# arturxe2/T-DEED

Hardware: AMD Instinct MI355X
Metric: clips/sec (L=100, 224^2, bf16) forward, per-frame logits (higher is better)
Workload: dtype bf16; 1 GPU; rny002_b8: rny002_gsf + ed_sgp_mixer n_layers=2 ks=7, L=100, 224x224, batch 8/GPU, inference forward, random-init weights; clips_per_gpu=8, parallelism=dp1 (clip-sharded, no collective), hip_graph=True, batches_in_flight=3, sub_batches_per_batch=1, dist_backend=none, dist_ranks=1, self_launched=False

## Files before the change

include/tdeed_hip.h:

```cpp
#ifndef TDEED_HIP_H
#define TDEED_HIP_H
#include <stdint.h>
#ifdef __cplusplus
extern "C" {
#endif

enum { TDEED_F32 = 0, TDEED_BF16 = 1 };
enum { TDEED_ACT_NONE = 0, TDEED_ACT_RELU = 1, TDEED_ACT_GELU = 2 };
enum { TDEED_OK = 0, TDEED_ERR_ARG = -1, TDEED_ERR_LAUNCH = -2, TDEED_ERR_RUNTIME = -3 };

const char* tdeed_last_error(void);
int tdeed_abi_version(void);
int tdeed_device_info(int dev, char* name64, int* n_cu, int* is_gfx950);

int tdeed_stem_fwd(const void* frames , int frames_f32,
                   int N, int H, int W, int crop_top, int crop_left,
                   int crop_h, int crop_w, int flip ,
                   const unsigned char* flip_mask ,
                   const float* w ,
                   const float* scale , const float* shift , void* out,
                   int relu , int dtype, void* stream);

int tdeed_stem_mfma_parts(int crop_h, int crop_w);
int tdeed_stem_mfma_fwd(const void* frames, int frames_f32, int N, int H, int W, int crop_top, int crop_left, int crop_h,
// ... 22 lines not shown
                      int gather_ho, int gather_wo, void* C2, long ldc2, int n2, int dtype, void* stream);

int tdeed_gemm_ws_sc_fits(int K, int Ks, int N, int dtype);
int tdeed_gemm_ws_sc_fwd(const void* A, long lda, const void* A0, long lda0, int k0, const float* a_scale,
                         int a_scale_rows, int M, int K, int N, const void* Wfrag, const float* scale,
                         const float* shift, const void* As, long ldas, int Ks, const void* Wsfrag,
                         const float* sscale, const float* sshift, int act, void* C, long ldc, int gather_stride,
                         int gather_hi, int gather_wi, int gather_ho, int gather_wo, void* C2, long ldc2, int n2,
                         int dtype, void* stream);

int tdeed_gconv3x3_parts(int Hi, int Wi, int C, int stride, int dtype);
int tdeed_gconv3x3_mfma_fits(int Hi, int Wi, int C, int stride);
int tdeed_gconv3x3_fwd(const void* x, int N, int Hi, int Wi, int C, int gw, int stride,
                       const float* w, const void* wfrag, const float* scale, const float* shift,
                       void* y, float* pooled, float* pooled_sq, const float* in_a, const float* in_b,
                       int relu , int dtype,
                       void* stream);

int tdeed_gemm_splitk_splits(int K);
int tdeed_gemm_splitk_partials(const void* A, long lda, int M, int K, int N, const void* W, long ldw, float* workspace,
                               void* stream);
int tdeed_gemm_splitk_fwd(const void* A, long lda, int M, int K, int N, const void* W, long ldw, const float* scale,
                          const float* shift, const void* R, long ldr, int act, void* C, long ldc,
                          float* workspace, void* stream);

int tdeed_se_gate_mfma_fits(int C, int R);
int tdeed_se_gate_mfma_fwd(const float* pooled, int n_parts, float inv_cnt, int N, int C, int R, const void* w1f,
                           const float* b1, const void* w2f, const float* b2, float* gate, void* stream);

int tdeed_gemm_rs_fits(int M, int K, int N);
int tdeed_gemm_rs_fwd(const void* A, long lda, const void* A0, long lda0, int k0, const float* a_scale, int a_scale_rows,
                      int M, int K, int N, const void* Wfrag, const float* scale, const float* shift, const void* R, long ldr,
                      int act, void* C, long ldc, void* C2, long ldc2, int n2, void* stream);

int tdeed_gemm_rs_grid(int M);
int tdeed_gemm_rs_stats_fwd(const void* A, long lda, const void* A0, long lda0, int k0, int M, int K, int N, const void* Wfrag,
                            void* C, long ldc, float* colpart, void* stream);

int tdeed_c1_gconv_set_debug(void* buf);
int tdeed_c1_gconv_fits(int Hi, int Wi, int Cin, int C, int stride);
int tdeed_c1_gconv_slab_tiles(int Hi, int Wi, int C, int stride);
int tdeed_c1_gconv_fwd(const void* x, const void* G, int Fp, int N, int Hi, int Wi, int Cin, int C, int gw, int stride,
                       const void* w1f, const float* s1, const float* h1, const void* wfrag, const float* scale,
                       const float* shift, void* y, float* pooled, void* stream);
int tdeed_c1_gconv_set_form(int form);
int tdeed_c1_gconv_slab_loop_fits(int Hi, int Wi, int Cin, int C, int stride);
int tdeed_c1_gconv_workgroups(int N, int Hi, int Wi, int Cin, int C, int stride);

int tdeed_c1_gconv_c3in_fits(int Hi, int Wi, int Cp, int C);
int tdeed_c1_gconv_c3in_fwd(const void* y2p, const void* scp, const float* gate, const void* w3f, const float* s3,
                            const float* h3, void* xs2, int N, int Hi, int Wi, int Cp, int C, int gw, const void* w1f,
                            const float* s1, const float* h1, const void* wfrag, const float* scale, const float* shift,
                            void* y, float* pooled, void* stream);

int tdeed_bneck_fits(int h, int w, int C, int R);
int tdeed_bneck_set_debug(void* buf);
int tdeed_bneck_fwd(const void* x, const void* G, int Fp, int N, int h, int w, int C, const void* w1f, const float* s1,
                    const float* h1, const void* w2f, const float* s2, const float* h2, const void* se_w1f,
                    const float* se_b1, const void* se_w2f, const float* se_b2, int R, const void* w3f, const float* s3,
                    const float* h3, void* out, void* out2, int n2,
                    int w2_tap_major ,
                    void* stream);
int tdeed_bneck_qtail_fits(int h, int w, int C, int F);
int tdeed_bneck_gs_fwd(const void* x, const void* gx, int ldx, const float* gate, const float* ysum, const float* xsum,
                       const float* cw1, const float* cb1, const float* cw2, const float* cb2, int T, int F, int Fp, int N,
                       int h, int w, int C, const void* w1f, const float* s1, const float* h1, const void* w2f,
                       const float* s2, const float* h2, const void* se_w1f, const float* se_b1, const void* se_w2f,
                       const float* se_b2, int R, const void* w3f, const float* s3, const float* h3, void* out, void* out2,
                       int n2, int w2_tap_major, const void* q_wqf, const float* q_bn, int q_F, float* Q, void* stream);


int tdeed_se_gate_fwd(const float* pooled, int n_parts, float inv_cnt, int N, int C, int R,
                      const float* w1t, const float* b1, const float* w2t, const float* b2,
                      float* gate, void* stream);

int tdeed_se_gate_bf16_fwd(const float* pooled, int n_parts, float inv_cnt, int N, int C, int R,
                           const void* w1p, const float* b1, const void* w2p, const float* b2,
                           float* gate, void* stream);

int tdeed_gsf_gate_fwd(const void* x, int B, int T, int h, int w, int C, int F,
                       const float* bn_scale, const float* bn_shift,
                       const float* wq ,
                       const void* wqf ,
                       const float* b3d ,
                       float* Q , float* gate, float* ysum, float* xsum,
                       int dtype, void* stream);
int tdeed_gsf_gate_sums_fwd(const void* x, int B, int T, int h, int w, int C, int F, const float* b3d, const float* Q,
                            float* gate, float* ysum, float* xsum, void* stream);
int tdeed_gsf_weight_fwd(const float* ysum, const float* xsum, int B, int T, int F, int hw,
                         const float* cw1 , const float* cb1, const float* cw2,
                         const float* cb2, float* fw , void* stream);
int tdeed_gsf_apply_fwd(const void* x, const float* gate, const float* fw , int B,
                        int T, int h, int w, int C, int F, int Fp, void* out, int dtype,
                        void* stream);

int tdeed_gsf_apply_fused_fwd(const void* x, const float* gate, const float* ysum, const float* xsum,
                              const float* cw1, const float* cb1, const float* cw2, const float* cb2, int B,
                              int T, int h, int w, int C, int F, int Fp, void* out, int dtype, void* stream);
int tdeed_gsf_blend_src_fwd(const void* x, const float* gate, const float* ysum, const float* xsum,
                            const float* cw1, const float* cb1, const float* cw2, const float* cb2, int B,
                            int T, int h, int w, int C, int F, int Fp, void* out, int dtype, void* stream);

int tdeed_avgpool_posenc_fwd(const void* x, int B, int T, int hw, int C, const float* temp_enc,
                             void* feat, float* rowstat, int dtype, int dtype_out , void* stream);

int tdeed_layernorm_fwd(const void* x, long ldx, int rows, int C, const float* w, const float* b,
// ... 248 lines not shown
```

t-deed_amd/_lib.py:

```python
import ctypes
import os
from ctypes import c_int, c_long, c_float, c_double, c_void_p, c_char_p, c_uint64, POINTER

import torch

CSRC = os.path.join(os.path.dirname(os.path.abspath(__file__)), "csrc")
LIB_PATH = os.path.join(CSRC, "libtdeed_hip.so")

F32, BF16 = 0, 1
ACT_NONE, ACT_RELU, ACT_GELU = 0, 1, 2


class HipLibraryMissing(RuntimeError):
    pass


class HipCallError(RuntimeError):
    pass


P = c_void_p
_SIGS = {
    "tdeed_abi_version": ([], c_int),
    "tdeed_device_info": ([c_int, c_char_p, POINTER(c_int), POINTER(c_int)], c_int),
    "tdeed_stem_fwd": ([P, c_int, c_int, c_int, c_int, c_int, c_int, c_int, c_int, c_int, P, P, P, P, P, c_int, c_int, P], c_int),
    "tdeed_augment_scratch_floats": ([c_int], c_long),
    "tdeed_augment_clips": ([P, c_int, c_int, c_int, c_int, c_int, c_int, c_int, c_int, c_int, P, P, P, P, P], c_int),
    "tdeed_mix_frames": ([P, P, P, c_int, c_long, P, P], c_int),
    "tdeed_avgpool_posenc_bwd": ([P, c_int, c_int, c_int, c_int, P, P, c_int, P], c_int),
    "tdeed_stem_mfma_parts": ([c_int, c_int], c_int),
    "tdeed_stem_mfma_fwd": ([P, c_int, c_int, c_int, c_int, c_int, c_int, c_int, c_int, c_int, P, P, P, P, P], c_int),
    "tdeed_stem_wgrad": ([P, c_int, c_int, c_int, c_int, c_int, c_int, c_int, c_int, c_int, P, P, P, P, c_int, P], c_int),
    "tdeed_stem_wgrad_bn_fits": ([c_int, c_int, c_int, c_int], c_int),
    "tdeed_stem_wgrad_bn": ([P, c_int, c_int, c_int, c_int, c_int, c_int, c_int, c_int, c_int, P, P, P, P, P, P, P, P, P, P], c_int),
    "tdeed_s1_front_parts": ([c_int, c_int, c_int], c_int),
    "tdeed_s1_front_fwd": ([P, c_int, c_int, c_int, c_int, c_int, c_int, c_int, c_int, P, P, P, c_int, P, P, P, P, P, P,
                            P, P, P, P, P, P, P], c_int),
    "tdeed_gemm_fwd": ([P, c_long, P, c_long, c_int, P, c_int, c_int, c_int, c_int, P, c_long, P, P, P, c_long,
                        c_int, P, c_long, c_int, c_int, c_int, c_int, c_int, P, P, c_long, c_int, c_int, c_int, P], c_int),
    "tdeed_gemm_ws_fits": ([c_int, c_int, c_int], c_int),
    "tdeed_gemm_ws_fwd": ([P, c_long, P, c_long, c_int, P, c_int, c_int, c_int, c_int, P, P, P, P, c_long,
                           c_int, P, c_long, c_int, c_int, c_int, c_int, c_int, P, c_long, c_int, c_int, P], c_int),
    "tdeed_gemm_ws_sc_fits": ([c_int, c_int, c_int, c_int], c_int),
    "tdeed_gemm_ws_sc_fwd": ([P, c_long, P, c_long, c_int, P, c_int, c_int, c_int, c_int, P, P, P, P, c_long, c_int, P, P, P,
                              c_int, P, c_long, c_int, c_int, c_int, c_int, c_int, P, c_long, c_int, c_int, P], c_int),
    "tdeed_gconv3x3_parts": ([c_int, c_int, c_int, c_int, c_int], c_int),
    "tdeed_gconv3x3_mfma_fits": ([c_int, c_int, c_int, c_int], c_int),
    "tdeed_gconv3x3_fwd": ([P, c_int, c_int, c_int, c_int, c_int, c_int, P, P, P, P, P, P, P, P, P, c_int, c_int, P], c_int),
    "tdeed_gemm_splitk_splits": ([c_int], c_int),
    "tdeed_gemm_splitk_fwd": ([P, c_long, c_int, c_int, c_int, P, c_long, P, P, P, c_long, c_int, P, c_long, P, P], c_int),
    "tdeed_se_gate_mfma_fits": ([c_int, c_int], c_int),
    "tdeed_se_gate_mfma_fwd": ([P, c_int, c_float, c_int, c_int, c_int, P, P, P, P, P, P], c_int),
    "tdeed_gemm_rs_fits": ([c_int, c_int, c_int], c_int),
    "tdeed_gemm_rs_grid": ([c_int], c_int),
    "tdeed_gemm_rs_stats_fwd": ([P, c_long, P, c_long, c_int, c_int, c_int, c_int, P, P, c_long, P, P], c_int),
    "tdeed_gemm_rs_fwd": ([P, c_long, P, c_long, c_int, P, c_int, c_int, c_int, c_int, P, P, P, P, c_long, c_int, P, c_long, P,
                           c_long, c_int, P], c_int),
    "tdeed_c1_gconv_set_debug": ([P], c_int),
    "tdeed_c1_gconv_fits": ([c_int, c_int, c_int, c_int, c_int], c_int),
    "tdeed_c1_gconv_slab_tiles": ([c_int, c_int, c_int, c_int], c_int),
    "tdeed_c1_gconv_fwd": ([P, P, c_int, c_int, c_int, c_int, c_int, c_int, c_int, c_int, P, P, P, P, P, P, P, P,
                            P], c_int),
    "tdeed_c1_gconv_set_form": ([c_int], c_int),
    "tdeed_c1_gconv_slab_loop_fits": ([c_int, c_int, c_int, c_int, c_int], c_int),
    "tdeed_c1_gconv_workgroups": ([c_int, c_int, c_int, c_int, c_int, c_int], c_int),
    "tdeed_c1_gconv_c3in_fits": ([c_int, c_int, c_int, c_int], c_int),
    "tdeed_c1_gconv_c3in_fwd": ([P, P, P, P, P, P, P, c_int, c_int, c_int, c_int, c_int, c_int, P, P, P, P, P, P, P, P,
                                 P], c_int),
    "tdeed_bneck_fits": ([c_int, c_int, c_int, c_int], c_int),
    "tdeed_bneck_set_debug": ([P], c_int),
    "tdeed_bneck_fwd": ([P, P, c_int, c_int, c_int, c_int, c_int, P, P, P, P, P, P, P, P, P, P, c_int, P, P, P, P, P, c_int,
                         c_int, P], c_int),
    "tdeed_bneck_gs_fwd": ([P, P, c_int, P, P, P, P, P, P, P, c_int, c_int, c_int, c_int, c_int, c_int, c_int, P, P, P, P, P, P, P,
                            P, P, P, c_int, P, P, P, P, P, c_int, c_int, P, P, c_int, P, P], c_int),
    "tdeed_bneck_qtail_fits": ([c_int, c_int, c_int, c_int], c_int),
    "tdeed_gsf_gate_sums_fwd": ([P, c_int, c_int, c_int, c_int, c_int, c_int, P, P, P, P, P, P], c_int),
    "tdeed_bn_slabs": ([c_long], c_int),
    "tdeed_bn_train_stats": ([P, c_long, c_int, P, P, c_float, c_float, P, P, P, P, P, P, P, c_int, P], c_int),
    "tdeed_bn_apply": ([P, c_long, c_int, P, P, P, c_int, P, c_int, P], c_int),
    "tdeed_bn_apply_slice": ([P, c_long, c_int, P, P, P, P, P, c_int, P, P, c_int, c_int, c_int, P], c_int),
    "tdeed_bn_apply2": ([P, c_long, c_int, P, P, P, P, P, c_int, P, c_int, P], c_int),
    "tdeed_bn_train_bwd": ([P, P, P, c_int, c_long, c_int, P, P, P, P, P, P, P, P, P, P, P, c_int, P], c_int),
    "tdeed_fold_rows": ([P, c_long, c_int, c_int, c_int, P, c_long, P], c_int),
    "tdeed_bn_finalize": ([P, P, c_long, c_int, c_long, c_int, P, P, c_float, c_float, P, P, P, P, P, P, P], c_int),
    "tdeed_pool_rows": ([P, P, c_int, c_int, c_int, P, P, c_int, P, c_int, P], c_int),
    "tdeed_se_train_fwd": ([P, c_int, c_int, c_int, P, P, P, P, P, P, P], c_int),
    "tdeed_se_train_bwd": ([P, P, P, c_int, c_int, c_int, P, P, P, P, P, P], c_int),
    "tdeed_scale_rows": ([P, P, P, c_float, c_int, c_int, c_int, P, P, P, c_int, P], c_int),
    "tdeed_gconv3x3_dgrad_stats": ([P, c_int, c_int, c_int, c_int, c_int, P, P, P, P, P, P, P, P, P, P, P], c_int),
    "tdeed_gconv3x3_bwd_stats_bands": ([c_int], c_int),
    "tdeed_gconv3x3_bwd_stats_fits": ([c_int, c_int, c_int, c_int, c_int], c_int),
    "tdeed_gconv3x3_bwd_stats": ([P, P, c_int, c_int, c_int, c_int, c_int, P, P, P, P, P, P, P, P, P, P, P, P, P], c_int),
    "tdeed_bn_bwd_masked_from_parts": ([P, P, c_long, c_int, P, P, P, P, P, P, P, c_long, c_int, P, P, c_int, P], c_int),
    "tdeed_narrow_conv1_bwd_fits": ([c_int, c_int], c_int),
    "tdeed_narrow_conv1_bwd_grid": ([c_long, c_int, c_int], c_int),
    "tdeed_narrow_conv1_bwd": ([P, P, c_long, c_int, c_int, P, P, P, P, P, P, P, P, P, c_long, c_int, c_int, P, c_int, P, P, P, P,
                                P, P, P], c_int),
    "tdeed_bn_sums_from_parts": ([P, P, c_long, c_int, c_int, P, P, P], c_int),
    "tdeed_se_bn_bwd_sums": ([P, P, c_int, c_int, c_int, P, P, P, P, c_int, P], c_int),
    "tdeed_se_bn_bwd_finalize": ([P, P, P, c_int, c_int, c_int, P, P, P], c_int),
    "tdeed_se_bn_bwd_apply": ([P, P, P, P, c_int, c_int, c_int, P, P, P, P, P, P, P, c_int, P], c_int),
    "tdeed_gemm_dgrad": ([P, c_long, c_int, c_int, c_int, P, c_long, P, c_long, c_int, c_int, P, c_long, P, c_long, c_int, P,
                          c_long, P, c_long, P, P, c_long, P, P, c_int, P], c_int),
    "tdeed_gemm_dgrad_rs": ([P, c_long, c_int, c_int, c_int, P, P, c_long, P, c_long, P, c_long, c_int, P, c_long, P, c_long, P, P,
                             P], c_int),
    "tdeed_gsf_add_cols_sink_parts": ([c_long, c_int, c_int], c_int),
    "tdeed_gsf_add_cols_sink": ([P, P, c_long, c_int, c_int, P, P, c_long, P, c_long, P, P, c_long, P, P, c_int, P], c_int),
    "tdeed_bn_bwd_from_parts": ([P, P, c_long, c_int, P, P, P, P, c_int, P, c_int, c_int, c_int, P, P, P, c_int, P], c_int),
    "tdeed_gconv_wgrad_slabs": ([c_long], c_int),
    "tdeed_gconv3x3_bwd": ([P, P, c_int, c_int, c_int, c_int, c_int, c_int, P, P, P, P, P, P, c_int, P], c_int),
    "tdeed_stride2_rows": ([P, P, c_int, c_int, c_int, c_int, c_int, c_int, P], c_int),
    "tdeed_loss2": ([P, c_int, c_int, c_int, c_int, c_int, P, P, P, P, c_int, P, c_float, P, P, P], c_int),
    "tdeed_reduce_strided": ([P, c_int, c_long, c_long, P, P], c_int),
    "tdeed_gsf_slice": ([P, c_long, c_int, c_int, c_int, P, c_int, P], c_int),
    "tdeed_gsf_bwd_scratch_floats": ([c_int, c_int, c_int, c_int], c_long),
    "tdeed_gsf_bwd_part_layout": ([c_int, c_int, c_int, c_int, P], c_int),
    "tdeed_sgp_gemm_ksteps": ([c_int], c_int),
    "tdeed_sgp_gemm_row_tiles": ([c_int, c_int], c_int),
    "tdeed_sgp_gemm_col_tiles": ([c_int, c_int], c_int),
    "tdeed_sgp_gemm_form": ([c_int, c_int, c_int, c_int, c_int], c_int),
    "tdeed_sgp_gemm_gn_gelu": ([P, c_int, c_int, c_int, P, c_int, P, P, c_int, c_float, P, P, c_int, P, c_int, c_int, P], c_int),
# ... 181 lines not shown
```

t-deed_amd/csrc/conv.hip:

```cpp
#include "common.h"

template <typename T, typename IN>
__global__ __launch_bounds__(256) void stem_kernel(const IN* __restrict__ frames, int H, int W,
                                                   int top, int left, int ch, int cw, int flip_all,
                                                   const unsigned char* __restrict__ flip_mask,
                                                   const float* __restrict__ w,
                                                   const float* __restrict__ scale,
                                                   const float* __restrict__ shift, T* __restrict__ out,
                                                   int Ho, int Wo, int relu) {
  __shared__ float tile[3][33][34];
  const int n = blockIdx.z;
  const int oy0 = blockIdx.y * 16, ox0 = blockIdx.x * 16;
  const int iy0 = oy0 * 2 - 1, ix0 = ox0 * 2 - 1;
  const float mean[3] = {0.485f, 0.456f, 0.406f};
  const float stdv[3] = {0.229f, 0.224f, 0.225f};
  const IN* src = frames + (long)n * 3 * H * W;
  const int flip = flip_mask ? (int)flip_mask[n] : flip_all;
  for (int i = threadIdx.x; i < 3 * 33 * 33; i += 256) {
    int c = i / (33 * 33);
    int r = i - c * 33 * 33;
    int y = r / 33, x = r - y * 33;
    int iy = iy0 + y, ix = ix0 + x;
    float v = 0.f;
    if (iy >= 0 && iy < ch && ix >= 0 && ix < cw) {
// ... 862 lines not shown
    fold[0][c] = c < C ? fa[j] : 0.f;
    fold[1][c] = c < C ? fb[j] : 0.f;
  }
  __syncthreads();
  GC_STAMP(1);
  bf16x8 xf[NT][KS1];
#pragma unroll
  for (int g = 0; g < NT; ++g)
#pragma unroll
    for (int ks = 0; ks < KS1; ++ks) {
      const u32x4 z = {0u, 0u, 0u, 0u};
      const u32x4 w = (poks[g] && 32 * ks + 8 * q < Cin) ? xv[g][ks] : z;
      xf[g][ks] = *reinterpret_cast<const bf16x8*>(&w);
    }
  auto conv1_pair = [&](int sl, int tlo) {
#pragma unroll
    for (int t = tlo; t < tlo + 2; ++t) {
      const f32x4 av = *reinterpret_cast<const f32x4*>(&fold[0][sl * 64 + t * 16 + 4 * q]);
      const f32x4 bv = *reinterpret_cast<const f32x4*>(&fold[1][sl * 64 + t * 16 + 4 * q]);
#pragma unroll
      for (int g = 0; g < NT; ++g) {
        if (wv + 4 * g >= ntl) break;
        f32x4 acc = {0.f, 0.f, 0.f, 0.f};
#pragma unroll
        for (int ks = 0; ks < KS1; ++ks) acc = __builtin_amdgcn_mfma_f32_16x16x32_bf16(w1r[t][ks], xf[g][ks], acc, 0, 0, 0);
        if (poks[g]) {
          bf16x4 o;
#pragma unroll
          for (int e = 0; e < 4; ++e) o[e] = (bf16_t)fmaxf(acc[e] * av[e] + bv[e], 0.f);
          *reinterpret_cast<bf16x4*>(tile + dsto[g] + t * 32) = o;
        }
      }
    }
  };
  for (int s = 0; s < nslabs_; ++s) {
    const int sn = min(s + 1, nslabs_ - 1);
    conv1_pair(s, 0);
    load_w1(sn, 0);
    conv1_pair(s, 2);
    if (s == 0) GC_STAMP(2);
    __syncthreads();
    if (s == 0) GC_STAMP(3);
    gconv_band_mma<STRIDE>(gw_, tile, red, redq, Wi, C, wfrag, scale, shift, y, pooled, nullptr, Ho, Wo, nbands, SCSP, PS, relu, n,
                           bnd, s, oy0, nrows_out);
    if (s == 0) GC_STAMP(4);
    load_w1(sn, 2);
    gw_ = gconv_load_w(wfrag, sn, SCSP);
    __syncthreads();
  }
  GC_STAMP(5);
  GC_STAMP(6);
}

static long long* g_c1g_dbg = nullptr;
extern "C" int tdeed_c1_gconv_set_debug(void* buf) { g_c1g_dbg = (long long*)buf; return TDEED_OK; }

extern "C" int tdeed_gconv3x3_mfma_fits(int Hi, int Wi, int C, int stride) {
  return gc_geom(Hi, Wi, C, stride).band > 0 ? 1 : 0;
}

extern "C" int tdeed_gconv3x3_parts(int Hi, int Wi, int C, int stride, int dtype) {
  if (dtype != TDEED_BF16) return 1;
  GcGeom g = gc_geom(Hi, Wi, C, stride);
  return g.band > 0 ? g.nbands : 1;
}

static int gconv3x3_launch(const void* x, int N, int Hi, int Wi, int C, int gw, int stride, const float* w, const void* wfrag,
                           const float* scale, const float* shift, void* y, float* pooled, float* pooled_sq, const float* in_a,
                           const float* in_b, int relu, int dtype, void* stream, const GcStat bst);
extern "C" int tdeed_gconv3x3_fwd(const void* x, int N, int Hi, int Wi, int C, int gw, int stride,
                                  const float* w, const void* wfrag, const float* scale, const float* shift,
                                  void* y, float* pooled, float* pooled_sq, const float* in_a, const float* in_b, int relu,
                                  int dtype, void* stream) {
  return gconv3x3_launch(x, N, Hi, Wi, C, gw, stride, w, wfrag, scale, shift, y, pooled, pooled_sq, in_a, in_b, relu, dtype,
                         stream, GcStat{nullptr, nullptr, nullptr, nullptr});
}
extern "C" int tdeed_gconv3x3_dgrad_stats(const void* dy, int N, int Hi, int Wi, int C, int gw, const void* wfrag_t,
                                          const float* one, const float* zero, void* dx, const void* bz, const float* bfa,
                                          const float* bfb, const float* bmean, float* part_s, float* part_q, void* stream) {
  TD_CHECK(bz && bfa && bfb && bmean && part_s && part_q && wfrag_t && one && zero, "gconv3x3_dgrad_stats: null pointer");
  TD_CHECK(tdeed_gconv3x3_mfma_fits(Hi, Wi, C, 1), "gconv3x3_dgrad_stats: %dx%dx%d is not served by the MFMA kernel", Hi, Wi, C);
  return gconv3x3_launch(dy, N, Hi, Wi, C, gw, 1, nullptr, wfrag_t, one, zero, dx, part_s, part_q, nullptr, nullptr, 0,
                         TDEED_BF16, stream, GcStat{(const bf16_t*)bz, bfa, bfb, bmean});
}
static int gconv3x3_launch(const void* x, int N, int Hi, int Wi, int C, int gw, int stride, const float* w, const void* wfrag,
                           const float* scale, const float* shift, void* y, float* pooled, float* pooled_sq, const float* in_a,
                           const float* in_b, int relu, int dtype, void* stream, const GcStat bst) {
  TD_CHECK(x && scale && shift && y && pooled, "gconv3x3: null pointer");
  TD_CHECK(!in_a == !in_b, "gconv3x3: in_a and in_b come together");
  TD_CHECK(!in_a || (dtype == TDEED_BF16 && wfrag), "gconv3x3: the on-load input affine exists in the bf16 MFMA kernel only");
  TD_CHECK(!pooled_sq || (dtype == TDEED_BF16 && wfrag), "gconv3x3: sums of squares come from the bf16 MFMA kernel only");
  TD_CHECK((gw == 8 || gw == 16) && C % gw == 0, "gconv3x3: group width %d / C %d unsupported", gw, C);
  TD_CHECK(stride == 1 || stride == 2, "gconv3x3: stride %d", stride);
  TD_CHECK(N > 0 && N <= 65535 && Hi > 0 && Wi > 0, "gconv3x3: bad sizes");
  hipStream_t st = (hipStream_t)stream;
  if (dtype == TDEED_F32) {
    TD_CHECK(w, "gconv3x3: fp32 path needs the packed fp32 weights");
    return gw == 8 ? launch_gconv<float, 8>(x, N, Hi, Wi, C, stride, w, scale, shift, y, pooled, relu, st)
                   : launch_gconv<float, 16>(x, N, Hi, Wi, C, stride, w, scale, shift, y, pooled, relu, st);
  }
  if (dtype == TDEED_BF16) {
    GcGeom g = gc_geom(Hi, Wi, C, stride);
    if (!wfrag || g.band <= 0) {
      TD_CHECK(w, "gconv3x3: no weights");
      TD_CHECK(!in_a, "gconv3x3: a row of %d px x %d ch does not fit LDS; no on-load input affine on the VALU path", Wi, C);
      return gw == 8 ? launch_gconv<bf16_t, 8>(x, N, Hi, Wi, C, stride, w, scale, shift, y, pooled, relu, st)
// ... 44 lines not shown
static bool c1g_slab_loop_wins(int ks1) { return ks1 == 2 || ks1 == 5; }
static bool c1g_slab_loop(int Hi, int Wi, int Cin, int C, int stride) {
  if (g_c1g_form == 0 || !tdeed_c1_gconv_slab_loop_fits(Hi, Wi, Cin, C, stride)) return false;
  return g_c1g_form == 1 || c1g_slab_loop_wins((Cin + 31) / 32);
}
extern "C" int tdeed_c1_gconv_workgroups(int N, int Hi, int Wi, int Cin, int C, int stride) {
  if (N <= 0 || !tdeed_c1_gconv_fits(Hi, Wi, Cin, C, stride)) return 0;
  const GcGeom g = gc_geom(Hi, Wi, C, stride);
  return N * g.nbands * (c1g_slab_loop(Hi, Wi, Cin, C, stride) ? 1 : g.nslabs);
}
extern "C" int tdeed_c1_gconv_fwd(const void* x, const void* G, int Fp, int N, int Hi, int Wi, int Cin, int C, int gw,
                                  int stride, const void* w1f, const float* s1, const float* h1, const void* wfrag,
                                  const float* scale, const float* shift, void* y, float* pooled, void* stream) {
  TD_CHECK(x && w1f && s1 && h1 && wfrag && scale && shift && y && pooled, "c1_gconv: null pointer");
  TD_CHECK((gw == 8 || gw == 16) && C % gw == 0, "c1_gconv: group width %d / C %d unsupported", gw, C);
  TD_CHECK(stride == 1 || stride == 2, "c1_gconv: stride %d", stride);
  TD_CHECK(N > 0 && N <= 65535 && tdeed_c1_gconv_fits(Hi, Wi, Cin, C, stride), "c1_gconv: Hi=%d Wi=%d Cin=%d C=%d unsupported",
           Hi, Wi, Cin, C);
  TD_CHECK(!G || (Fp % 8 == 0 && Fp > 0 && Fp <= Cin), "c1_gconv: bad splice width %d", Fp);
  const GcGeom g = gc_geom(Hi, Wi, C, stride);
  const int Ho = (Hi - 1) / stride + 1, Wo = (Wi - 1) / stride + 1;
  const bool slabs = c1g_slab_loop(Hi, Wi, Cin, C, stride);
  dim3 grid((unsigned)((long)g.nbands * (slabs ? 1 : g.nslabs) * N));
  const size_t smem = (size_t)g.rows_in * (Wi + 2) * g.PS;
  hipStream_t st = (hipStream_t)stream;
  const int KS1 = (Cin + 31) / 32;
#define TD_C1G(Sv, Kv)                                                                                                       \
  hipLaunchKernelGGL((c1_gconv_mfma_kernel<Sv, Kv>), grid, dim3(256), smem, st, (const bf16_t*)x, (const bf16_t*)G,           \
                     G ? Fp : 0, Hi, Wi, Cin, C, (const bf16x8*)w1f, s1, h1, (const bf16x8*)wfrag, scale, shift, (bf16_t*)y,  \
                     pooled, Ho, Wo, g.band, g.nbands, g.CSP, g.PS, g.rows_in, 1, g_c1g_dbg, C3In{})
#define TD_C1G_K(Sv)                                                                                                       \
  do {                                                                                                                     \
    if (KS1 == 1) TD_C1G(Sv, 1); else if (KS1 == 2) TD_C1G(Sv, 2); else if (KS1 == 4) TD_C1G(Sv, 4);                      \
    else TD_C1G(Sv, 5);                                                                                                    \
  } while (0)
  if (slabs) {
#define TD_C1G_SL(Kv)                                                                                                       \
  hipLaunchKernelGGL((c1_gconv_slab_loop_kernel<2, Kv>), grid, dim3(256), smem, st, (const bf16_t*)x, (const bf16_t*)G,        \
                     G ? Fp : 0, Hi, Wi, Cin, C, (const bf16x8*)w1f, s1, h1, (const bf16x8*)wfrag, scale, shift, (bf16_t*)y,  \
                     pooled, Ho, Wo, g.band, g.nbands, g.CSP, g.PS, g.rows_in, 1, g_c1g_dbg)
    if (KS1 == 2) TD_C1G_SL(2); else TD_C1G_SL(5);
#undef TD_C1G_SL
  } else if (stride == 2) TD_C1G_K(2); else TD_C1G_K(1);
#undef TD_C1G_K
#undef TD_C1G
  TD_LAUNCH_CHECK("c1_gconv");
  return TDEED_OK;
}

extern "C" int tdeed_c1_gconv_c3in_fits(int Hi, int Wi, int Cp, int C) {
  if (Cp < 8 || Cp > 32 || Cp % 8 != 0 || C > 64 || !tdeed_c1_gconv_fits(Hi, Wi, Cp, C, 2)) return 0;
  return gc_geom(Hi, Wi, C, 2).nslabs == 1 ? 1 : 0;
}
extern "C" int tdeed_c1_gconv_c3in_fwd(const void* y2p, const void* scp, const float* gate, const void* w3f, const float* s3,
                                       const float* h3, void* xs2, int N, int Hi, int Wi, int Cp, int C, int gw,
                                       const void* w1f, const float* s1, const float* h1, const void* wfrag,
                                       const float* scale, const float* shift, void* y, float* pooled, void* stream) {
  TD_CHECK(y2p && scp && gate && w3f && s3 && h3, "c1_gconv_c3in: null pointer (the producer's operands)");
  TD_CHECK(w1f && s1 && h1 && wfrag && scale && shift && y && pooled, "c1_gconv_c3in: null pointer");
  TD_CHECK((gw == 8 || gw == 16) && C % gw == 0, "c1_gconv_c3in: group width %d / C %d unsupported", gw, C);
  TD_CHECK(N > 0 && N <= 65535 && tdeed_c1_gconv_c3in_fits(Hi, Wi, Cp, C), "c1_gconv_c3in: Hi=%d Wi=%d Cp=%d C=%d unsupported",
           Hi, Wi, Cp, C);
  const GcGeom g = gc_geom(Hi, Wi, C, 2);
  const int Ho = (Hi - 1) / 2 + 1, Wo = (Wi - 1) / 2 + 1;
  dim3 grid((unsigned)((long)g.nbands * N));
  const size_t smem = (size_t)g.rows_in * (Wi + 2) * g.PS;
  const C3In c3{(const bf16_t*)y2p, (const bf16_t*)scp, gate, (const bf16x8*)w3f, s3, h3, (bf16_t*)xs2};
  hipLaunchKernelGGL((c1_gconv_mfma_kernel<2, 1, true>), grid, dim3(256), smem, (hipStream_t)stream, (const bf16_t*)nullptr,
                     (const bf16_t*)nullptr, 0, Hi, Wi, Cp, C, (const bf16x8*)w1f, s1, h1, (const bf16x8*)wfrag, scale, shift,
                     (bf16_t*)y, pooled, Ho, Wo, g.band, g.nbands, g.CSP, g.PS, g.rows_in, 1, g_c1g_dbg, c3);
  TD_LAUNCH_CHECK("c1_gconv_c3in");
  return TDEED_OK;
}

#define SE_FPB 4
__global__ __launch_bounds__(256) void se_gate_kernel(const float* __restrict__ pooled, int n_parts, float inv_cnt,
                                                      int N, int C, int R, const float* __restrict__ w1t,
                                                      const float* __restrict__ b1,
                                                      const float* __restrict__ w2t,
                                                      const float* __restrict__ b2, float* __restrict__ gate) {
  extern __shared__ float sm[];
  float* sp = sm;
  float* shid = sm + SE_FPB * C;
  const int f0 = blockIdx.x * SE_FPB;
  for (int i = threadIdx.x; i < SE_FPB * C; i += 256) {
    const int f = i / C, c = i - f * C;
    float v = 0.f;
    if (f0 + f < N) {
      const float* src = pooled + ((long)(f0 + f) * n_parts) * C + c;
      for (int q = 0; q < n_parts; ++q) v += src[(long)q * C];
    }
    sp[i] = v * inv_cnt;
  }
  __syncthreads();
  {
    const int RP = R <= 32 ? 32 : (R <= 64 ? 64 : (R <= 128 ? 128 : 256));
    const int nsl = 256 / RP;
    const int j = threadIdx.x % RP, sl = threadIdx.x / RP;
    float a[SE_FPB];
#pragma unroll
    for (int f = 0; f < SE_FPB; ++f) a[f] = 0.f;
    if (j < R) {
      const int cper = (C + nsl - 1) / nsl;
      const int c0 = sl * cper, c1 = min(C, c0 + cper);
#pragma unroll 8
      for (int c = c0; c < c1; ++c) {
        const float wv_ = w1t[(long)c * R + j];
#pragma unroll
        for (int f = 0; f < SE_FPB; ++f) a[f] = fmaf(sp[f * C + c], wv_, a[f]);
      }
    }
    float* part = shid + SE_FPB * R;
    if (j < R) {
#pragma unroll
      for (int f = 0; f < SE_FPB; ++f) part[(sl * SE_FPB + f) * R + j] = a[f];
    }
    __syncthreads();
    for (int i = threadIdx.x; i < SE_FPB * R; i += 256) {
      float v = 0.f;
      for (int q = 0; q < nsl; ++q) v += part[q * SE_FPB * R + i];
// ... 482 lines not shown
```

t-deed_amd/ops.py:

```python
import ctypes

import torch

from . import _lib
from ._lib import call, ptr, stream_ptr, dtype_code, ACT_NONE, ACT_RELU, ACT_GELU


def _chk(t, name, dtype=None):
    if t is None:
        return
    if not t.is_cuda:
        raise RuntimeError(f"{name} must be a GPU tensor (tdeed_amd has no CPU path)")
    if not t.is_contiguous():
        raise RuntimeError(f"{name} must be contiguous")
    if dtype is not None and t.dtype != dtype:
        raise TypeError(f"{name}: expected {dtype}, got {t.dtype}")


def _flip_args(flip, N):
    if isinstance(flip, torch.Tensor):
        m = flip.to(torch.uint8).contiguous()
        if m.numel() != N or not m.is_cuda:
            raise ValueError(f"flip mask must hold one flag per frame on the GPU ({m.numel()} vs {N})")
        return 0, m
# ... 82 lines not shown
    lda = A.shape[-1] if lda is None else lda
    if out is None:
        out = torch.empty((M, N), dtype=A.dtype, device=A.device)
    ldc = N if ldc is None else ldc
    g = gather if gather is not None else (1, 0, 0, 0, 0)
    call("tdeed_gemm_fwd", ptr(A), lda, ptr(A0), (A0.shape[-1] if A0 is not None else 0), k0,
         ptr(a_scale), a_scale_rows, M, K, N, ptr(W), W.shape[1], ptr(scale), ptr(shift),
         ptr(residual), (residual.shape[-1] if residual is not None else 0), act, ptr(out), ldc,
         g[0], g[1], g[2], g[3], g[4], ptr(colpart), *_out2(out2, A), int(bool(out2_pre)), dtype_code(A.dtype), stream_ptr())
    return out


def c1_gconv_fits(Hi, Wi, Cin, C, stride):
    return _lib.load().tdeed_c1_gconv_fits(Hi, Wi, Cin, C, stride) != 0


def c1_gconv_slab_loop_fits(Hi, Wi, Cin, C, stride):
    lib = _lib.load()
    if not hasattr(lib, "tdeed_c1_gconv_slab_loop_fits"):
        return False
    return lib.tdeed_c1_gconv_slab_loop_fits(Hi, Wi, Cin, C, stride) != 0


def c1_gconv_set_form(form):
    call("tdeed_c1_gconv_set_form", form)


def c1_gconv_workgroups(N, Hi, Wi, Cin, C, stride):
    return _lib.load().tdeed_c1_gconv_workgroups(N, Hi, Wi, Cin, C, stride)


def c1_gconv_slab_tiles(Hi, Wi, C, stride):
    return _lib.load().tdeed_c1_gconv_slab_tiles(Hi, Wi, C, stride)


def c1_gconv(x, w1f, s1, h1, wfrag, scale, shift, gw, stride, C, G=None, out=None, pooled=None):
    _chk(x, "x", torch.bfloat16); _chk(G, "G", torch.bfloat16)
    N, Hi, Wi, Cin = x.shape
    Ho, Wo = (Hi - 1) // stride + 1, (Wi - 1) // stride + 1
    if out is None:
        out = torch.empty((N, Ho, Wo, C), dtype=x.dtype, device=x.device)
    if pooled is None:
        pooled = torch.empty((N, gconv3x3_parts(Hi, Wi, C, stride, x.dtype), C), dtype=torch.float32, device=x.device)
    call("tdeed_c1_gconv_fwd", ptr(x), ptr(G), (G.shape[-1] if G is not None else 0), N, Hi, Wi, Cin, C, gw, stride, ptr(w1f),
         ptr(s1), ptr(h1), ptr(wfrag), ptr(scale), ptr(shift), ptr(out), ptr(pooled), stream_ptr())
    return out, pooled


def c1_gconv_c3in_fits(Hi, Wi, Cp, C):
    lib = _lib.load()
    if not hasattr(lib, "tdeed_c1_gconv_c3in_fits"):
        return False
    return lib.tdeed_c1_gconv_c3in_fits(Hi, Wi, Cp, C) != 0


def c1_gconv_c3in(y2p, scp, gate, w3frag, s3, h3, w1f, s1, h1, wfrag, scale, shift, gw, C, xs2=None, out=None, pooled=None):
    _chk(y2p, "y2p", torch.bfloat16); _chk(scp, "scp", torch.bfloat16); _chk(gate, "gate", torch.float32)
    _chk(xs2, "xs2", torch.bfloat16)
    N, Hi, Wi, Cp = y2p.shape
    Ho, Wo = (Hi - 1) // 2 + 1, (Wi - 1) // 2 + 1
    if tuple(scp.shape) != (N, Hi, Wi, Cp) or gate.numel() != N * Cp or (xs2 is not None and xs2.numel() != N * Ho * Wo * Cp):
        raise ValueError(f"c1_gconv_c3in: y2p {tuple(y2p.shape)}, scp {tuple(scp.shape)}, gate {tuple(gate.shape)}, "
                         f"xs2 {None if xs2 is None else tuple(xs2.shape)} do not belong together")
    if out is None:
        out = torch.empty((N, Ho, Wo, C), dtype=y2p.dtype, device=y2p.device)
    if pooled is None:
        pooled = torch.empty((N, gconv3x3_parts(Hi, Wi, C, 2, y2p.dtype), C), dtype=torch.float32, device=y2p.device)
    call("tdeed_c1_gconv_c3in_fwd", ptr(y2p), ptr(scp), ptr(gate), ptr(w3frag), ptr(s3), ptr(h3), ptr(xs2), N, Hi, Wi, Cp, C, gw,
         ptr(w1f), ptr(s1), ptr(h1), ptr(wfrag), ptr(scale), ptr(shift), ptr(out), ptr(pooled), stream_ptr())
    return out, pooled


def bneck_fits(h, w, C, R):
    return _lib.load().tdeed_bneck_fits(h, w, C, R) != 0


def bneck(x, w1f, s1, h1, w2f, s2, h2, se_w1f, se_b1, se_w2f, se_b2, R, w3f, s3, h3, G=None, out=None, out2=None,
          w2_tap_major=True):
    _chk(x, "x", torch.bfloat16); _chk(G, "G", torch.bfloat16); _chk(out2, "out2", torch.bfloat16)
    N, h, w, C = x.shape
    if out is None:
        out = torch.empty_like(x)
    call("tdeed_bneck_fwd", ptr(x), ptr(G), (G.shape[-1] if G is not None else 0), N, h, w, C, ptr(w1f), ptr(s1),
         ptr(h1), ptr(w2f), ptr(s2), ptr(h2), ptr(se_w1f), ptr(se_b1), ptr(se_w2f), ptr(se_b2), R, ptr(w3f), ptr(s3), ptr(h3),
         ptr(out), ptr(out2), (out2.shape[-1] if out2 is not None else 0), int(bool(w2_tap_major)), stream_ptr())
    return out


def bneck_gs(x, gx, gate, ysum, xsum, cw1, cb1, cw2, cb2, T, F, Fp, w1f, s1, h1, w2f, s2, h2, se_w1f, se_b1, se_w2f, se_b2, R,
             w3f, s3, h3, out=None, out2=None, w2_tap_major=True, qtail=None):
    _chk(x, "x", torch.bfloat16); _chk(gx, "gx", torch.bfloat16); _chk(out2, "out2", torch.bfloat16)
    N, h, w, C = x.shape
    if out is None:
        out = torch.empty_like(x)
    call("tdeed_bneck_gs_fwd", ptr(x), ptr(gx), gx.shape[-1], ptr(gate), ptr(ysum), ptr(xsum), ptr(cw1), ptr(cb1), ptr(cw2),
         ptr(cb2), T, F, Fp, N, h, w, C, ptr(w1f), ptr(s1), ptr(h1), ptr(w2f), ptr(s2), ptr(h2), ptr(se_w1f), ptr(se_b1),
         ptr(se_w2f), ptr(se_b2), R, ptr(w3f), ptr(s3), ptr(h3), ptr(out), ptr(out2),
         (out2.shape[-1] if out2 is not None else 0), int(bool(w2_tap_major)),
         *((ptr(qtail[0]), ptr(qtail[1]), int(qtail[2]), ptr(qtail[3])) if qtail is not None else (None, None, 0, None)),
         stream_ptr())
    return out


def bneck_qtail_fits(h, w, C, F):
    return _lib.load().tdeed_bneck_qtail_fits(h, w, C, F) != 0

# ... 816 lines not shown
```

Baseline: 5776 clips/s.

## Add band-walking c3in fused gconv kernel that streams consecutive bands per workgroup

Adds a new kernel variant of the fused c3-input 1x1+grouped-conv stage in which each workgroup walks a run of consecutive row bands instead of handling one band. It prefetches the next band's inputs into registers while the current band runs the grouped conv. It also carries the overlapping halo row forward in LDS, so that row is not reloaded and recomputed. The default routing uses runs of up to five bands. This cuts workgroup count and per-band setup (weight and BN loads, halo recompute), at the cost of fewer workgroups in flight and a serial chain inside each workgroup.

```diff
diff --git a/include/tdeed_hip.h b/include/tdeed_hip.h
--- a/include/tdeed_hip.h
+++ b/include/tdeed_hip.h
@@ -98,6 +98,9 @@
                             const float* h3, void* xs2, int N, int Hi, int Wi, int Cp, int C, int gw, const void* w1f,
                             const float* s1, const float* h1, const void* wfrag, const float* scale, const float* shift,
                             void* y, float* pooled, void* stream);
+int tdeed_c1_gconv_c3in_set_walk(int walk);
+int tdeed_c1_gconv_c3in_walk(int Hi, int Wi, int Cp, int C);
+int tdeed_c1_gconv_c3in_workgroups(int N, int Hi, int Wi, int Cp, int C);
 
 int tdeed_bneck_fits(int h, int w, int C, int R);
 int tdeed_bneck_set_debug(void* buf);
diff --git a/t-deed_amd/_lib.py b/t-deed_amd/_lib.py
--- a/t-deed_amd/_lib.py
+++ b/t-deed_amd/_lib.py
@@ -67,6 +67,9 @@
     "tdeed_c1_gconv_c3in_fits": ([c_int, c_int, c_int, c_int], c_int),
     "tdeed_c1_gconv_c3in_fwd": ([P, P, P, P, P, P, P, c_int, c_int, c_int, c_int, c_int, c_int, P, P, P, P, P, P, P, P,
                                  P], c_int),
+    "tdeed_c1_gconv_c3in_set_walk": ([c_int], c_int),
+    "tdeed_c1_gconv_c3in_walk": ([c_int, c_int, c_int, c_int], c_int),
+    "tdeed_c1_gconv_c3in_workgroups": ([c_int, c_int, c_int, c_int, c_int], c_int),
     "tdeed_bneck_fits": ([c_int, c_int, c_int, c_int], c_int),
     "tdeed_bneck_set_debug": ([P], c_int),
     "tdeed_bneck_fwd": ([P, P, c_int, c_int, c_int, c_int, c_int, P, P, P, P, P, P, P, P, P, P, c_int, P, P, P, P, P, c_int,
diff --git a/t-deed_amd/csrc/conv.hip b/t-deed_amd/csrc/conv.hip
--- a/t-deed_amd/csrc/conv.hip
+++ b/t-deed_amd/csrc/conv.hip
@@ -938,6 +938,211 @@
   GC_STAMP(6);
 }
 
+#define C3W_NPF 4
+template <int CSP>
+__global__ __launch_bounds__(256, 3) void c1_gconv_c3in_walk_kernel(int Hi, int Wi, int Cin, int C, const bf16x8* __restrict__ w1f,
+                                                            const float* __restrict__ s1, const float* __restrict__ h1,
+                                                            const bf16x8* __restrict__ wfrag, const float* __restrict__ scale,
+                                                            const float* __restrict__ shift, bf16_t* __restrict__ y,
+                                                            float* __restrict__ pooled, int Ho, int Wo, int band, int nbands,
+                                                            int walk, long long* dbg, const C3In c3) {
+  constexpr int PS = CSP * 2 + 16;
+  extern __shared__ __attribute__((aligned(16))) unsigned char tile[];
+  __shared__ float red[4][32];
+  __shared__ float redq[4][32];
+  __shared__ __attribute__((aligned(16))) float f1[2][64];
+  __shared__ __attribute__((aligned(16))) float f2[2][64];
+  __shared__ __attribute__((aligned(16))) float f3[3][32];
+  __shared__ __attribute__((aligned(16))) bf16x8 wl[6][64];
+  GC_STAMP(0);
+  const long lid = xcd_logical_id(blockIdx.x, gridDim.x);
+  const int nruns = (nbands + walk - 1) / walk;
+  int n, run;
+  td_split(lid, nruns, n, run);
+  const int b0 = run * walk, b1 = min(b0 + walk, nbands);
+  const int WP = Wi + 2;
+  const int tid = threadIdx.x, lane = tid & 63, wv = __builtin_amdgcn_readfirstlane(tid >> 6);
+  const int pl = lane & 15, q = lane >> 4;
+  const int nts = CSP >> 4;
+  const int k8 = 8 * q;
+  const bool kok = k8 < Cin;
+  const int kc = min(k8, Cin - 8);
+  const bf16_t* yn = c3.y2p + (long)n * Hi * Wi * Cin;
+  const bf16_t* rn = c3.scp + (long)n * Hi * Wi * Cin;
+  bf16_t* xsn = c3.xs2 ? c3.xs2 + (long)n * Ho * Wo * Cin : nullptr;
+  const IDiv dwi(Wi);
+  struct Bg { int oy0, nrows_out, iy0, nrow_used, r_lo, npx, ntl; };
+  auto geom = [&](int b, bool first) {
+    Bg g;
+    g.oy0 = b * band;
+    g.nrows_out = min(band, Ho - g.oy0);
+    g.iy0 = g.oy0 * 2 - 1;
+    g.nrow_used = (g.nrows_out - 1) * 2 + 3;
+    g.r_lo = first ? max(g.iy0, 0) : g.iy0 + 1;
+    g.npx = (min(g.iy0 + g.nrow_used, Hi) - g.r_lo) * Wi;
+    g.ntl = (g.npx + 15) >> 4;
+    return g;
+  };
+  auto request = [&](const Bg& g, int tb, u32x4 (&yf)[C3W_NPF], u32x4 (&rf)[C3W_NPF]) {
+#pragma unroll
+    for (int i = 0; i < C3W_NPF; ++i) {
+      const int t0 = tb + 4 * i;
+      const int p = t0 * 16 + pl;
+      int rr, cc;
+      dwi.divmod((t0 < g.ntl && p < g.npx) ? p : 0, rr, cc);
+      const unsigned o = (unsigned)(((g.r_lo + rr) * Wi + cc) * Cin + kc) * 2u;
+      yf[i] = *reinterpret_cast<const u32x4*>(reinterpret_cast<const unsigned char*>(yn) + o);
+      rf[i] = *reinterpret_cast<const u32x4*>(reinterpret_cast<const unsigned char*>(rn) + o);
+    }
+  };
+  Bg cur = geom(b0, true);
+  u32x4 yf[C3W_NPF], rf[C3W_NPF];
+  request(cur, wv, yf, rf);
+  auto load_gw = [&]() {
+    constexpr int pairs = CSP >= 32 ? CSP >> 5 : 1;
+    const unsigned char* wu = reinterpret_cast<const unsigned char*>(wfrag + (CSP >= 32 ? (wv % pairs) * 2 * 5 * 64 : 0));
+    unsigned lo = (unsigned)lane * 16u;
+    asm volatile("" : "+v"(lo));
+    GcW w;
+#pragma unroll
+    for (int ks = 0; ks < 5; ++ks) {
+      w.a[ks] = *reinterpret_cast<const bf16x8*>(wu + ks * 1024 + lo);
+      w.b[ks] = CSP >= 32 ? *reinterpret_cast<const bf16x8*>(wu + (5 + ks) * 1024 + lo) : w.a[ks];
+    }
+    return w;
+  };
+  GcW gw_;
+  {
+    const int i0 = tid, i1 = min(tid + 256, 6 * 64 - 1);
+    const bf16x8 wv0 = w1f[(long)min(i0 >> 6, nts - 1) * 64 + (i0 & 63)];
+    const bf16x8 wv1 = c3.w3f[i1 - 256];
+    const int c = tid & 63, cc = min(c, C - 1), c3c = min(tid & 31, Cin - 1);
+    const bool ok = c < C, ok3 = (tid & 31) < Cin;
+    const float v1a = s1[cc], v1b = h1[cc], v2a = scale[cc], v2b = shift[cc];
+    const float v3g = c3.gate[(long)n * Cin + c3c], v3a = c3.s3[c3c], v3b = c3.h3[c3c];
+    c1g_zero_halo(tile, cur.nrow_used, Hi, Wi, PS, cur.iy0);
+    if (tid < 64) {
+      f1[0][c] = ok ? v1a : 0.f;
+      f1[1][c] = ok ? v1b : 0.f;
+      f2[0][c] = ok ? v2a : 0.f;
+      f2[1][c] = ok ? v2b : 0.f;
+    } else if (tid < 96) {
+      f3[0][tid & 31] = v3g;
+      f3[1][tid & 31] = ok3 ? v3a : 1.f;
+      f3[2][tid & 31] = ok3 ? v3b : 0.f;
+    }
+    wl[i0 >> 6][i0 & 63] = wv0;
+    if (tid < 128) wl[4 + (tid >> 6)][tid & 63] = wv1;
+  }
+  __syncthreads();
+  GC_STAMP(1);
+  auto compute = [&](const Bg& g, int tb, const u32x4 (&yfi)[C3W_NPF], const u32x4 (&rfi)[C3W_NPF]) {
+    float g8[8], sc3[8], sh3[8];
+#pragma unroll
+    for (int e4 = 0; e4 < 8; e4 += 4) {
+      const f32x4 gv = *reinterpret_cast<const f32x4*>(&f3[0][kc + e4]);
+      const f32x4 sv = *reinterpret_cast<const f32x4*>(&f3[1][k8 + e4]), hv = *reinterpret_cast<const f32x4*>(&f3[2][k8 + e4]);
+#pragma unroll
+      for (int e = 0; e < 4; ++e) {
+        g8[e4 + e] = gv[e];
+        sc3[e4 + e] = sv[e];
+        sh3[e4 + e] = hv[e];
+      }
+    }
+    f32x4 a1[4], b1[4];
+    bf16x8 w1r[4];
+    const bf16x8 w3a = wl[4][lane], w3b = wl[5][lane];
+#pragma unroll
+    for (int t = 0; t < 4; ++t) {
+      w1r[t] = wl[t][lane];
+      a1[t] = *reinterpret_cast<const f32x4*>(&f1[0][t * 16 + 4 * q]);
+      b1[t] = *reinterpret_cast<const f32x4*>(&f1[1][t * 16 + 4 * q]);
+    }
+#pragma unroll
+    for (int i = 0; i < C3W_NPF; ++i) {
+      const int t0 = tb + 4 * i;
+      if (t0 >= g.ntl) break;
+      const int p = t0 * 16 + pl;
+      const bool pok = p < g.npx;
+      int rr, col;
+      dwi.divmod(pok ? p : 0, rr, col);
+      const bf16x8 y8 = *reinterpret_cast<const bf16x8*>(&yfi[i]), r8 = *reinterpret_cast<const bf16x8*>(&rfi[i]);
+      bf16x8 a8;
+#pragma unroll
+      for (int e = 0; e < 8; ++e) {
+        float f = (float)y8[e];
+        f *= g8[e];
+        a8[e] = (bf16_t)f;
+      }
+      const u32x4 zero4 = {0u, 0u, 0u, 0u};
+      const u32x4 am = (pok && kok) ? *reinterpret_cast<const u32x4*>(&a8) : zero4;
+      const f32x4 z4 = {0.f, 0.f, 0.f, 0.f};
+      const f32x4 c0 = __builtin_amdgcn_mfma_f32_16x16x32_bf16(w3a, *reinterpret_cast<const bf16x8*>(&am), z4, 0, 0, 0);
+      const f32x4 c1 = __builtin_amdgcn_mfma_f32_16x16x32_bf16(w3b, *reinterpret_cast<const bf16x8*>(&am), z4, 0, 0, 0);
+      float v[8];
+#pragma unroll
+      for (int r = 0; r < 4; ++r) {
+        v[r] = c0[r] * sc3[r] + sh3[r];
+        v[4 + r] = c1[r] * sc3[4 + r] + sh3[4 + r];
+      }
+      bf16x8 o8;
+#pragma unroll
+      for (int e = 0; e < 8; ++e) {
+        v[e] += (float)r8[e];
+        v[e] = fmaxf(v[e], 0.f);
+        o8[e] = (bf16_t)v[e];
+      }
+      const u32x4 xm = kok ? *reinterpret_cast<const u32x4*>(&o8) : zero4;
+      const bf16x8 xf = *reinterpret_cast<const bf16x8*>(&xm);
+      const int row = g.r_lo + rr;
+      if (xsn && pok && kok && !((row | col) & 1) && (row >> 1) >= g.oy0 && (row >> 1) < g.oy0 + g.nrows_out)
+        *reinterpret_cast<u32x4*>(xsn + ((long)(row >> 1) * Wo + (col >> 1)) * Cin + k8) = xm;
+      unsigned char* dst = tile + ((long)(row - g.iy0) * WP + col + 1) * PS + 8 * q;
+#pragma unroll
+      for (int t = 0; t < 4; ++t) {
+        if (t < nts) {
+          const f32x4 acc = __builtin_amdgcn_mfma_f32_16x16x32_bf16(w1r[t], xf, z4, 0, 0, 0);
+          if (pok) {
+            bf16x4 o;
+#pragma unroll
+            for (int e = 0; e < 4; ++e) o[e] = (bf16_t)fmaxf(acc[e] * a1[t][e] + b1[t][e], 0.f);
+            *reinterpret_cast<bf16x4*>(dst + t * 32) = o;
+          }
+        }
+      }
+    }
+  };
+  const int rowchunks = (WP * PS) >> 4;
+  for (int b = b0; b < b1; ++b) {
+    TD_ISSUE_FENCE();
+    const int rz = Hi - cur.iy0;
+    if (b != b0 && rz < cur.nrow_used)
+      for (int i = tid; i < rowchunks; i += 256)
+        *reinterpret_cast<u32x4*>(tile + rz * (WP * PS) + i * 16) = (u32x4){0u, 0u, 0u, 0u};
+    compute(cur, wv, yf, rf);
+    for (int tb = wv + 4 * C3W_NPF; tb < cur.ntl; tb += 4 * C3W_NPF) {
+      request(cur, tb, yf, rf);
+      compute(cur, tb, yf, rf);
+    }
+    const Bg nxt = geom(min(b + 1, b1 - 1), false);
+    gw_ = load_gw();
+    request(nxt, wv, yf, rf);
+    if (b == b0) GC_STAMP(2);
+    if (b == b0 + 1) GC_STAMP(4);
+    __syncthreads();
+    __builtin_amdgcn_s_waitcnt(0x0F70 | (2 * C3W_NPF));
+    gconv_band_mma<2>(gw_, tile, red, redq, Wi, C, wfrag, f2[0], f2[1], y, pooled, nullptr, Ho, Wo, nbands, CSP, PS, 1, n, b, 0,
+                      cur.oy0, cur.nrows_out);
+    for (int i = tid; i < rowchunks; i += 256)
+      *reinterpret_cast<u32x4*>(tile + i * 16) = *reinterpret_cast<const u32x4*>(tile + (cur.nrow_used - 1) * (WP * PS) + i * 16);
+    __syncthreads();
+    if (b == b0) GC_STAMP(3);
+    if (b == b0 + 1) GC_STAMP(5);
+    cur = nxt;
+  }
+  GC_STAMP(6);
+}
+
 static long long* g_c1g_dbg = nullptr;
 extern "C" int tdeed_c1_gconv_set_debug(void* buf) { g_c1g_dbg = (long long*)buf; return TDEED_OK; }
 
@@ -1088,6 +1293,33 @@
   if (Cp < 8 || Cp > 32 || Cp % 8 != 0 || C > 64 || !tdeed_c1_gconv_fits(Hi, Wi, Cp, C, 2)) return 0;
   return gc_geom(Hi, Wi, C, 2).nslabs == 1 ? 1 : 0;
 }
+#define C3IN_WALK_ROUTED 5
+static int g_c3in_walk = 0;
+extern "C" int tdeed_c1_gconv_c3in_set_walk(int walk) {
+  TD_CHECK(walk >= 0 && walk <= 65535, "c1_gconv_c3in_set_walk: %d (0 routed, 1 per band, k >= 2 runs of k bands)", walk);
+  g_c3in_walk = walk;
+  return TDEED_OK;
+}
+extern "C" int tdeed_c1_gconv_c3in_walk(int Hi, int Wi, int Cp, int C) {
+  if (!tdeed_c1_gconv_c3in_fits(Hi, Wi, Cp, C)) return 0;
+  if ((long)Hi * Wi * Cp * 2 >= (1L << 31)) return 1;
+  const int nb = gc_geom(Hi, Wi, C, 2).nbands;
+  return C3IN_WALK_ROUTED < nb ? C3IN_WALK_ROUTED : nb;
+}
+static int c3in_walk_in_force(int Hi, int Wi, int Cp, int C) {
+  static int env = -1;
+  if (env < 0) { const char* e = getenv("TDEED_C3IN_WALK"); env = e ? atoi(e) : 0; if (env < 0) env = 0; }
+  const int forced = g_c3in_walk ? g_c3in_walk : env;
+  if (forced == 0) return tdeed_c1_gconv_c3in_walk(Hi, Wi, Cp, C);
+  if ((long)Hi * Wi * Cp * 2 >= (1L << 31)) return 1;
+  const int nb = gc_geom(Hi, Wi, C, 2).nbands;
+  return forced < nb ? forced : nb;
+}
+extern "C" int tdeed_c1_gconv_c3in_workgroups(int N, int Hi, int Wi, int Cp, int C) {
+  if (N <= 0 || !tdeed_c1_gconv_c3in_fits(Hi, Wi, Cp, C)) return 0;
+  const int nb = gc_geom(Hi, Wi, C, 2).nbands, walk = c3in_walk_in_force(Hi, Wi, Cp, C);
+  return N * ((nb + walk - 1) / walk);
+}
 extern "C" int tdeed_c1_gconv_c3in_fwd(const void* y2p, const void* scp, const float* gate, const void* w3f, const float* s3,
                                        const float* h3, void* xs2, int N, int Hi, int Wi, int Cp, int C, int gw,
                                        const void* w1f, const float* s1, const float* h1, const void* wfrag,
@@ -1102,6 +1334,18 @@
   dim3 grid((unsigned)((long)g.nbands * N));
   const size_t smem = (size_t)g.rows_in * (Wi + 2) * g.PS;
   const C3In c3{(const bf16_t*)y2p, (const bf16_t*)scp, gate, (const bf16x8*)w3f, s3, h3, (bf16_t*)xs2};
+  const int walk = c3in_walk_in_force(Hi, Wi, Cp, C);
+  if (walk >= 2) {
+    dim3 wgrid((unsigned)((long)((g.nbands + walk - 1) / walk) * N));
+#define TD_C3W(CSPv)                                                                                                        \
+  hipLaunchKernelGGL((c1_gconv_c3in_walk_kernel<CSPv>), wgrid, dim3(256), smem, (hipStream_t)stream, Hi, Wi,  \
+                     Cp, C, (const bf16x8*)w1f, s1, h1, (const bf16x8*)wfrag, scale, shift, (bf16_t*)y, pooled, Ho, Wo,       \
+                     g.band, g.nbands, walk, g_c1g_dbg, c3)
+    if (g.CSP == 64) TD_C3W(64); else if (g.CSP == 32) TD_C3W(32); else TD_C3W(16);
+#undef TD_C3W
+    TD_LAUNCH_CHECK("c1_gconv_c3in_walk");
+    return TDEED_OK;
+  }
   hipLaunchKernelGGL((c1_gconv_mfma_kernel<2, 1, true>), grid, dim3(256), smem, (hipStream_t)stream, (const bf16_t*)nullptr,
                      (const bf16_t*)nullptr, 0, Hi, Wi, Cp, C, (const bf16x8*)w1f, s1, h1, (const bf16x8*)wfrag, scale, shift,
                      (bf16_t*)y, pooled, Ho, Wo, g.band, g.nbands, g.CSP, g.PS, g.rows_in, 1, g_c1g_dbg, c3);
diff --git a/t-deed_amd/ops.py b/t-deed_amd/ops.py
--- a/t-deed_amd/ops.py
+++ b/t-deed_amd/ops.py
@@ -158,6 +158,18 @@
     if not hasattr(lib, "tdeed_c1_gconv_c3in_fits"):
         return False
     return lib.tdeed_c1_gconv_c3in_fits(Hi, Wi, Cp, C) != 0
+
+
+def c1_gconv_c3in_set_walk(walk):
+    call("tdeed_c1_gconv_c3in_set_walk", walk)
+
+
+def c1_gconv_c3in_walk(Hi, Wi, Cp, C):
+    return _lib.load().tdeed_c1_gconv_c3in_walk(Hi, Wi, Cp, C)
+
+
+def c1_gconv_c3in_workgroups(N, Hi, Wi, Cp, C):
+    return _lib.load().tdeed_c1_gconv_c3in_workgroups(N, Hi, Wi, Cp, C)
 
 
 def c1_gconv_c3in(y2p, scp, gate, w3frag, s3, h3, w1f, s1, h1, wfrag, scale, shift, gw, C, xs2=None, out=None, pooled=None):
```

New measurement: 5933 clips/s (median of 6 runs). 1.03x the previous value.
